# syshin1014/wssdl_bus

Hardware: AMD Instinct MI355X
Metric: images/sec (train step, 600x1000) (higher is better)
Workload: dtype f32; 1 GPU; resnet50_joint_b8; backbone=ResNet-50, image=600x1000, images_per_gpu=8, supervised_per_gpu=4, weak_per_gpu=4, mode=joint, parallelism=image-parallel dp1, RCCL grad all-reduce, sampling_rng=device, fused_rpn_softmax=True, padded_rois=False, miopen_find=True, miopen_find_db=wssdl_bus_amd/miopen_db (HIP.3_5_0_20250912-42-1199-g2584e35062), miopen_searched=True

## Files before the change

### wssdl_bus_amd/csrc/plumbing/rowbn.hip

```cpp
#include <hip/hip_runtime.h>
#include <stdint.h>
#include <type_traits>

#define PLUMB_API extern "C" __attribute__((visibility("default")))

namespace {

constexpr int BLOCK = 256;
constexpr int MAX_PARTIAL_BLOCKS = 1024;

typedef float float4v __attribute__((ext_vector_type(4)));

template <int MASK>
__device__ __forceinline__ unsigned mask_roi(long long r, int div) {
    return MASK == 2 ? (unsigned)r % (unsigned)div : (unsigned)r / (unsigned)div;
}

__device__ __forceinline__ float bn_affine(float x, float sc, float sh) { return __builtin_fmaf(x, sc, sh); }
__device__ __forceinline__ float bn_dx(float ka, float u, float k0, float k1, float x) {
    return __builtin_fmaf(-k1, x, __builtin_fmaf(ka, u, -k0));
}
__device__ __forceinline__ void dot_rows2(double &q, float v0, float w0, float v1, float w1) {
#pragma clang fp contract(off)
    const double p1 = (double)v1 * (double)w1;
    q += __builtin_fma((double)v0, (double)w0, p1);
}
__device__ __forceinline__ void dot_row(double &q, float v, float w) { q = __builtin_fma((double)v, (double)w, q); }
__device__ __forceinline__ void acc_rows2(double &s, double &q, float v0, float w0, float v1, float w1) {
    s += (double)v0 + (double)v1;
    dot_rows2(q, v0, w0, v1, w1);
}
__device__ __forceinline__ void acc_row(double &s, double &q, float v, float w) {
    s += (double)v;
    dot_row(q, v, w);
}

template <int MASK>
__device__ __forceinline__ bool row_live(const float *__restrict__ mask, long long r, int div) {
    return MASK ? mask[mask_roi<MASK>(r, div)] != 0.0f : true;
}

__device__ __forceinline__ float4v load4(const float *__restrict__ p, long long r, int C, int c4, bool on) {
    const float4v zero4 = {0, 0, 0, 0};
    return on ? reinterpret_cast<const float4v *>(p + (size_t)r * C)[c4] : zero4;
}

__device__ __forceinline__ void store4(float *__restrict__ p, long long r, int C, int c4, float4v v) {
    reinterpret_cast<float4v *>(p + (size_t)r * C)[c4] = v;
}

struct EntryGrad {
    const float *dys;
    const int *possel;
    int per, R;
};

template <bool ENTRY>
__device__ __forceinline__ float4v load_dy(const float *__restrict__ dy, const EntryGrad &e, long long r, int C, int c4,
                                           bool on = true) {
    const float4v zero4 = {0, 0, 0, 0};
    if (!on) return zero4;
    const float4v g = reinterpret_cast<const float4v *>(dy + (size_t)r * C)[c4];
    if (!ENTRY) return g;
    const unsigned roi = (unsigned)r / (unsigned)e.per, p = (unsigned)r - roi * (unsigned)e.per;
    const int slot = e.possel[p];
    float4v d = zero4;
    if (slot >= 0) d = reinterpret_cast<const float4v *>(e.dys + ((size_t)slot * e.R + roi) * C)[c4] + zero4;
    return g + d;
}

struct Slab {
    int C4, L, RS, lc, lr;
    long long r0, r1;
    __device__ __forceinline__ Slab(long long M, int C, long long rows_per_block) {
        C4 = C >> 2;
        L = C4 < BLOCK ? C4 : BLOCK;
        RS = BLOCK / L;
        lc = threadIdx.x % L;
        lr = threadIdx.x / L;
        r0 = (long long)blockIdx.x * rows_per_block;
        r1 = r0 + rows_per_block < M ? r0 + rows_per_block : M;
    }
};

__device__ __forceinline__ void slab_reduce(const Slab &b, int C, int c4, const double (&s)[4], const double (&q)[4],
                                            double (*red)[8], double *__restrict__ out) {
    const int t = threadIdx.x;
    __syncthreads();
#pragma unroll
    for (int j = 0; j < 4; ++j) { red[t][j] = s[j]; red[t][4 + j] = q[j]; }
    __syncthreads();
    if (b.lr == 0) {
#pragma unroll
        for (int j = 0; j < 4; ++j) {
            double ss = 0.0, qq = 0.0;
            for (int k = 0; k < b.RS; ++k) { ss += red[k * b.L + b.lc][j]; qq += red[k * b.L + b.lc][4 + j]; }
            out[c4 * 4 + j] = ss;
            out[C + c4 * 4 + j] = qq;
        }
    }
}

struct Term {
    float4v v, w, w2;
};

template <int MASK, class F>
__device__ __forceinline__ void slab_walk(const Slab &b, int C, const float *__restrict__ mask, int div, F &f,
                                          double (*red)[8], double *__restrict__ out,
                                          double *__restrict__ out2 = nullptr) {
    const int RS = b.RS;
    for (int cc = 0; cc * b.L < b.C4; ++cc) {
        const int c4 = cc * b.L + b.lc;
        double s[4] = {0, 0, 0, 0}, q[4] = {0, 0, 0, 0}, q2[4] = {0, 0, 0, 0};
        f.setup(c4);
        if (b.lr < RS) {
            long long r = b.r0 + b.lr;
#pragma unroll 1
            for (; r + RS < b.r1; r += 2 * RS) {
                const bool live0 = row_live<MASK>(mask, r, div), live1 = row_live<MASK>(mask, r + RS, div);
                if (!F::VISITS_DEAD && !live0 && !live1) continue;
                const typename F::Row a0 = f.load(r, c4, live0), a1 = f.load(r + RS, c4, live1);
                const Term t0 = f.finish(a0, r, c4, live0), t1 = f.finish(a1, r + RS, c4, live1);
#pragma unroll
                for (int j = 0; j < 4; ++j) {
                    const float v0 = live0 ? t0.v[j] : 0.0f, v1 = live1 ? t1.v[j] : 0.0f;
                    acc_rows2(s[j], q[j], v0, live0 ? t0.w[j] : 0.0f, v1, live1 ? t1.w[j] : 0.0f);
                    if (F::TWO_Q) dot_rows2(q2[j], v0, live0 ? t0.w2[j] : 0.0f, v1, live1 ? t1.w2[j] : 0.0f);
                }
            }
            for (; r < b.r1; r += RS) {
                const bool live = row_live<MASK>(mask, r, div);
                if (!F::VISITS_DEAD && !live) continue;
                const Term t = f.finish(f.load(r, c4, live), r, c4, live);
                if (live) {
#pragma unroll
                    for (int j = 0; j < 4; ++j) {
                        acc_row(s[j], q[j], t.v[j], t.w[j]);
                        if (F::TWO_Q) dot_row(q2[j], t.v[j], t.w2[j]);
                    }
                }
            }
        }
        slab_reduce(b, C, c4, s, q, red, out);
        if (F::TWO_Q) slab_reduce(b, C, c4, s, q2, red, out2);
    }
}

template <int MODE, bool RELU, bool ENTRY>
struct PartialCols {
    static constexpr bool VISITS_DEAD = false, TWO_Q = false;
    const float *x, *dy, *scale, *shift;
    int C;
    EntryGrad eg;
    float4v sc, sh;
    struct Row {
        float4v a, g;
    };
    __device__ __forceinline__ void setup(int c4) {
        if (MODE == 1 && RELU) {
            sc = reinterpret_cast<const float4v *>(scale)[c4];
            sh = reinterpret_cast<const float4v *>(shift)[c4];
        }
    }
    __device__ __forceinline__ Row load(long long r, int c4, bool live) const {
        Row w = {load4(x, r, C, c4, live), {0, 0, 0, 0}};
        if (MODE == 1) w.g = load_dy<ENTRY>(dy, eg, r, C, c4, live);
        return w;
    }
    __device__ __forceinline__ Term finish(const Row &w, long long, int, bool) const {
        Term t = {w.a, w.a, {0, 0, 0, 0}};
        if (MODE == 1) {
            t.v = w.g;
#pragma unroll
            for (int j = 0; j < 4; ++j)
                if (RELU && !(bn_affine(w.a[j], sc[j], sh[j]) > 0.0f)) t.v[j] = 0.0f;
        }
        return t;
    }
};

template <int MODE, bool RELU, int MASK, bool ENTRY = false>
__global__ __launch_bounds__(BLOCK) void rowbn_partial_kernel(
    const float *__restrict__ x, const float *__restrict__ dy, const float *__restrict__ scale,
    const float *__restrict__ shift, long long M, int C, long long rows_per_block,
    double *__restrict__ partial, const float *__restrict__ mask, int per, EntryGrad eg = EntryGrad()) {
    __shared__ double red[BLOCK][8];
    const Slab b(M, C, rows_per_block);
    PartialCols<MODE, RELU, ENTRY> f = {x, dy, scale, shift, C, eg};
    slab_walk<MASK>(b, C, mask, per, f, red, partial + (size_t)blockIdx.x * 2 * C);
}

constexpr int FIN_COLS = 16, FIN_GROUPS = 64;

__device__ __forceinline__ void finish_reduce(const double *__restrict__ partial, int nblocks, int C,
                                              int c, int grp, double (*red)[FIN_COLS][2], double &s,
                                              double &q) {
    double ss = 0.0, qq = 0.0;
    if (c < C)
        for (int b = grp; b < nblocks; b += FIN_GROUPS) {
            ss += partial[(size_t)b * 2 * C + c];
            qq += partial[(size_t)b * 2 * C + C + c];
        }
    red[grp][threadIdx.x % FIN_COLS][0] = ss;
    red[grp][threadIdx.x % FIN_COLS][1] = qq;
    __syncthreads();
    s = 0.0;
    q = 0.0;
    if (grp == 0)
        for (int g = 0; g < FIN_GROUPS; ++g) {
            s += red[g][threadIdx.x][0];
            q += red[g][threadIdx.x][1];
        }
}

__device__ __forceinline__ double live_rows(const float *__restrict__ mask, int n_rois, int per, long long M,
                                            double *scratch ) {
    if (!mask) return (double)M;
    double c = 0.0;
    for (int i = threadIdx.x; i < n_rois; i += FIN_COLS * FIN_GROUPS) c += mask[i] != 0.0f ? 1.0 : 0.0;
    __syncthreads();
    scratch[threadIdx.x] = c;
    __syncthreads();
    double t = 0.0;
    for (int i = 0; i < FIN_COLS * FIN_GROUPS; ++i) t += scratch[i];
    __syncthreads();
    t *= (double)per;
    return t < 1.0 ? 1.0 : t;
}

struct Running {
    float *mean, *var;
    float momentum;
    long long *batches;
};

__device__ __forceinline__ float running_update(float r, float stat, double unbias, double mom) {
#pragma clang fp contract(off)
    const double t = (double)stat * unbias;
    const double d = t - (double)r;
    const double p = mom * d;
    return (float)((double)r + p);
}

__global__ __launch_bounds__(FIN_COLS * FIN_GROUPS) void rowbn_fwd_finish_kernel(
    const double *__restrict__ partial, int nblocks, int C, long long M,
    const float *__restrict__ weight, const float *__restrict__ bias, float eps,
    float *__restrict__ mean, float *__restrict__ var, float *__restrict__ rstd,
    float *__restrict__ scale, float *__restrict__ shift, const float *__restrict__ mask, int n_rois, int per,
    float *__restrict__ count, Running run) {
    __shared__ double red[FIN_GROUPS][FIN_COLS][2];
    const int grp = threadIdx.x / FIN_COLS;
    const int c = blockIdx.x * FIN_COLS + threadIdx.x % FIN_COLS;
    const double Mn = live_rows(mask, n_rois, per, M, &red[0][0][0]);
    if (blockIdx.x == 0 && threadIdx.x == 0) {
        if (count) count[0] = (float)Mn;
        if (run.batches) run.batches[0] = run.batches[0] + 1;
    }
    double s, q;
    finish_reduce(partial, nblocks, C, c, grp, red, s, q);
    if (grp != 0 || c >= C) return;
    const double mu = s / Mn;
    double v = q / Mn - mu * mu;
    if (v < 0.0) v = 0.0;
    const float rs = (float)(1.0 / sqrt(v + (double)eps));
    const float scl = rs * weight[c];
    mean[c] = (float)mu;
    var[c] = (float)v;
    rstd[c] = rs;
    scale[c] = scl;
    shift[c] = bias[c] - (float)mu * scl;
    const double mom = (double)run.momentum;
    if (run.mean) run.mean[c] = running_update(run.mean[c], (float)mu, 1.0, mom);
    if (run.var) run.var[c] = running_update(run.var[c], (float)v, Mn / (Mn - 1.0 > 1.0 ? Mn - 1.0 : 1.0), mom);
}

__global__ __launch_bounds__(FIN_COLS * FIN_GROUPS) void rowbn_bwd_finish_kernel(
    const double *__restrict__ partial, int nblocks, int C, long long M,
    const float *__restrict__ weight, const float *__restrict__ mean,
    const float *__restrict__ rstd, float *__restrict__ dweight, float *__restrict__ dbias,
    float *__restrict__ coef, const float *__restrict__ mask, int n_rois, int per) {
    __shared__ double red[FIN_GROUPS][FIN_COLS][2];
    const int grp = threadIdx.x / FIN_COLS;
    const int c = blockIdx.x * FIN_COLS + threadIdx.x % FIN_COLS;
    const double Mn = live_rows(mask, n_rois, per, M, &red[0][0][0]);
    double sg, sgx;
    finish_reduce(partial, nblocks, C, c, grp, red, sg, sgx);
    if (grp != 0 || c >= C) return;
    const double mu = mean[c], rs = rstd[c], w = weight[c];
    const double sum_g_xhat = (sgx - mu * sg) * rs;
    const double a = w * rs;
    const double k1 = a * rs * sum_g_xhat / Mn;
    const double k0 = a * sg / Mn - k1 * mu;
    dweight[c] = (float)sum_g_xhat;
    dbias[c] = (float)sg;
    coef[c] = (float)a;
    coef[C + c] = (float)k0;
    coef[2 * C + c] = (float)k1;
}

template <bool RELU, int MASK>
__global__ __launch_bounds__(BLOCK) void rowbn_apply_fwd_kernel(
    const float *__restrict__ x, const float *__restrict__ scale, const float *__restrict__ shift,
    long long total4, int C4, float *__restrict__ y, const float *__restrict__ mask, int per) {
    for (long long i = (long long)blockIdx.x * BLOCK + threadIdx.x; i < total4;
         i += (long long)gridDim.x * BLOCK) {
        const int c4 = (int)(i % C4);
        if (MASK && mask[mask_roi<MASK>(i / C4, per)] == 0.0f) {
            const float4v zero4 = {0, 0, 0, 0};
            reinterpret_cast<float4v *>(y)[i] = zero4;
            continue;
        }
        const float4v a = reinterpret_cast<const float4v *>(x)[i];
        const float4v sc = reinterpret_cast<const float4v *>(scale)[c4];
        const float4v sh = reinterpret_cast<const float4v *>(shift)[c4];
        float4v o;
#pragma unroll
        for (int j = 0; j < 4; ++j) {
            float v = bn_affine(a[j], sc[j], sh[j]);
            if (RELU) v = v > 0.0f ? v : 0.0f;
            o[j] = v;
        }
        reinterpret_cast<float4v *>(y)[i] = o;
    }
}

template <bool RELU, int MASK, bool ENTRY = false>
__global__ __launch_bounds__(BLOCK) void rowbn_apply_bwd_kernel(
    const float *__restrict__ x, const float *__restrict__ dy, const float *__restrict__ scale,
    const float *__restrict__ shift, const float *__restrict__ coef, long long total4, int C4,
    float *__restrict__ dx, const float *__restrict__ mask, int per, EntryGrad eg = EntryGrad()) {
    const int C = C4 * 4;
    for (long long i = (long long)blockIdx.x * BLOCK + threadIdx.x; i < total4;
         i += (long long)gridDim.x * BLOCK) {
        const int c4 = (int)(i % C4);
        if (MASK && mask[mask_roi<MASK>(i / C4, per)] == 0.0f) {
            const float4v zero4 = {0, 0, 0, 0};
            reinterpret_cast<float4v *>(dx)[i] = zero4;
            continue;
        }
        const float4v a = reinterpret_cast<const float4v *>(x)[i];
        const float4v g = ENTRY ? load_dy<true>(dy, eg, i / C4, C, c4) : reinterpret_cast<const float4v *>(dy)[i];
        const float4v ka = reinterpret_cast<const float4v *>(coef)[c4];
        const float4v k0 = reinterpret_cast<const float4v *>(coef + C)[c4];
        const float4v k1 = reinterpret_cast<const float4v *>(coef + 2 * C)[c4];
        float4v sc = {0, 0, 0, 0}, sh = {0, 0, 0, 0};
        if (RELU) {
            sc = reinterpret_cast<const float4v *>(scale)[c4];
            sh = reinterpret_cast<const float4v *>(shift)[c4];
        }
        float4v o;
#pragma unroll
        for (int j = 0; j < 4; ++j) {
            float u = g[j];
            if (RELU && !(bn_affine(a[j], sc[j], sh[j]) > 0.0f)) u = 0.0f;
            o[j] = bn_dx(ka[j], u, k0[j], k1[j], a[j]);
        }
        reinterpret_cast<float4v *>(dx)[i] = o;
    }
}


__device__ __forceinline__ void acc_rows2_loose(double &s, double &q, float v0, float w0, float v1, float w1) {
    s += (double)v0 + (double)v1;
    q += (double)v0 * (double)w0 + (double)v1 * (double)w1;
}
__device__ __forceinline__ void acc_row_loose(double &s, double &q, float v, float w) {
    s += (double)v;
    q += (double)v * (double)w;
}

template <bool DUAL, int MASK>
__global__ __launch_bounds__(BLOCK) void rowbn_join_fwd_kernel(
    const float *__restrict__ x3, const float *__restrict__ sc3, const float *__restrict__ sh3,
    const float *__restrict__ other, const float *__restrict__ sco, const float *__restrict__ sho, long long M,
    int C, long long rows_per_block, float *__restrict__ out, double *__restrict__ partial,
    const float *__restrict__ mask, int div) {
    __shared__ double red[BLOCK][8];
    const Slab b(M, C, rows_per_block);
    double *pout = partial + (size_t)blockIdx.x * 2 * C;
    for (int cc = 0; cc * b.L < b.C4; ++cc) {
        const int c4 = cc * b.L + b.lc;
        double s[4] = {0, 0, 0, 0}, q[4] = {0, 0, 0, 0};
        const float4v k3 = reinterpret_cast<const float4v *>(sc3)[c4], h3 = reinterpret_cast<const float4v *>(sh3)[c4];
        float4v ko = {0, 0, 0, 0}, ho = {0, 0, 0, 0};
        if (DUAL) {
            ko = reinterpret_cast<const float4v *>(sco)[c4];
            ho = reinterpret_cast<const float4v *>(sho)[c4];
        }
        auto join = [&](float a, float o, int j, bool live) {
            const float t = live ? bn_affine(a, k3[j], h3[j]) : 0.0f;
            const float u = DUAL ? (live ? bn_affine(o, ko[j], ho[j]) : 0.0f) : o;
            return t + u;
        };
        if (b.lr < b.RS) {
            const int RS = b.RS;
            long long r = b.r0 + b.lr;
#pragma unroll 1
            for (; r + RS < b.r1; r += 2 * RS) {
                const bool live0 = row_live<MASK>(mask, r, div), live1 = row_live<MASK>(mask, r + RS, div);
                const float4v a0 = load4(x3, r, C, c4, live0), a1 = load4(x3, r + RS, C, c4, live1);
                const float4v o0 = load4(other, r, C, c4, !DUAL || live0), o1 = load4(other, r + RS, C, c4, !DUAL || live1);
                float4v y0, y1;
#pragma unroll
                for (int j = 0; j < 4; ++j) {
                    y0[j] = join(a0[j], o0[j], j, live0);
                    y1[j] = join(a1[j], o1[j], j, live1);
                    const float v0 = live0 ? y0[j] : 0.0f, v1 = live1 ? y1[j] : 0.0f;
                    acc_rows2_loose(s[j], q[j], v0, v0, v1, v1);
                }
                store4(out, r, C, c4, y0);
                store4(out, r + RS, C, c4, y1);
            }
            for (; r < b.r1; r += RS) {
                const bool live0 = row_live<MASK>(mask, r, div);
                const float4v a0 = load4(x3, r, C, c4, live0), o0 = load4(other, r, C, c4, !DUAL || live0);
                float4v y0;
#pragma unroll
                for (int j = 0; j < 4; ++j) {
                    y0[j] = join(a0[j], o0[j], j, live0);
                    if (live0) acc_row_loose(s[j], q[j], y0[j], y0[j]);
                }
                store4(out, r, C, c4, y0);
            }
        }
        slab_reduce(b, C, c4, s, q, red, pout);
    }
}

template <bool DUAL, bool RES>
struct JoinBwdCols {
    static constexpr bool VISITS_DEAD = true, TWO_Q = DUAL;
    const float *xo, *dy, *scn, *shn, *coef, *dres, *x3, *xs;
    float *g;
    int C;
    float4v sc, sh, ka, k0, k1;
    struct Row {
        float4v x, d, e, a, b;
    };
    __device__ __forceinline__ void setup(int c4) {
        sc = reinterpret_cast<const float4v *>(scn)[c4];
        sh = reinterpret_cast<const float4v *>(shn)[c4];
        ka = reinterpret_cast<const float4v *>(coef)[c4];
        k0 = reinterpret_cast<const float4v *>(coef + C)[c4];
        k1 = reinterpret_cast<const float4v *>(coef + 2 * C)[c4];
    }
    __device__ __forceinline__ Row load(long long r, int c4, bool live) const {
        return {load4(xo, r, C, c4, live), load4(dy, r, C, c4, live), load4(dres, r, C, c4, RES),
                load4(x3, r, C, c4, live), load4(xs, r, C, c4, DUAL && live)};
    }
    __device__ __forceinline__ Term finish(const Row &w, long long r, int c4, bool live) const {
        float4v o;
#pragma unroll
        for (int j = 0; j < 4; ++j) {
            float u = w.d[j];
            if (!(bn_affine(w.x[j], sc[j], sh[j]) > 0.0f)) u = 0.0f;
            const float dx = live ? bn_dx(ka[j], u, k0[j], k1[j], w.x[j]) : 0.0f;
            o[j] = RES ? dx + w.e[j] : dx;
        }
        store4(g, r, C, c4, o);
        return {o, w.a, w.b};
    }
};

template <bool DUAL, bool RES, int MASK>
__global__ __launch_bounds__(BLOCK) void rowbn_join_bwd_kernel(
    const float *__restrict__ xo, const float *__restrict__ dy, const float *__restrict__ scn,
    const float *__restrict__ shn, const float *__restrict__ coef, const float *__restrict__ dres,
    const float *__restrict__ x3, const float *__restrict__ xs, long long M, int C, long long rows_per_block,
    float *__restrict__ g, double *__restrict__ partial3, double *__restrict__ partials,
    const float *__restrict__ mask, int div) {
    __shared__ double red[BLOCK][8];
    const Slab b(M, C, rows_per_block);
    JoinBwdCols<DUAL, RES> f = {xo, dy, scn, shn, coef, dres, x3, xs, g, C};
    slab_walk<MASK>(b, C, mask, div, f, red, partial3 + (size_t)blockIdx.x * 2 * C,
                    DUAL ? partials + (size_t)blockIdx.x * 2 * C : nullptr);
}

template <int MASK>
__global__ __launch_bounds__(BLOCK) void rowbn_apply_bwd_dual_kernel(
    const float *__restrict__ x3, const float *__restrict__ xs, const float *__restrict__ g,
    const float *__restrict__ coef3, const float *__restrict__ coefs, long long total4, int C4,
    float *__restrict__ dx3, float *__restrict__ dxs, const float *__restrict__ mask, int div) {
    const int C = C4 * 4;
    for (long long i = (long long)blockIdx.x * BLOCK + threadIdx.x; i < total4;
         i += (long long)gridDim.x * BLOCK) {
        const int c4 = (int)(i % C4);
        if (MASK && mask[mask_roi<MASK>(i / C4, div)] == 0.0f) {
            const float4v zero4 = {0, 0, 0, 0};
            reinterpret_cast<float4v *>(dx3)[i] = zero4;
            reinterpret_cast<float4v *>(dxs)[i] = zero4;
            continue;
        }
        const float4v a = reinterpret_cast<const float4v *>(x3)[i];
        const float4v e = reinterpret_cast<const float4v *>(xs)[i];
        const float4v u = reinterpret_cast<const float4v *>(g)[i];
        const float4v ka3 = reinterpret_cast<const float4v *>(coef3)[c4], kas = reinterpret_cast<const float4v *>(coefs)[c4];
        const float4v k03 = reinterpret_cast<const float4v *>(coef3 + C)[c4], k0s = reinterpret_cast<const float4v *>(coefs + C)[c4];
        const float4v k13 = reinterpret_cast<const float4v *>(coef3 + 2 * C)[c4], k1s = reinterpret_cast<const float4v *>(coefs + 2 * C)[c4];
        float4v o3, os;
#pragma unroll
        for (int j = 0; j < 4; ++j) {
            o3[j] = bn_dx(ka3[j], u[j], k03[j], k13[j], a[j]);
            os[j] = bn_dx(kas[j], u[j], k0s[j], k1s[j], e[j]);
        }
        reinterpret_cast<float4v *>(dx3)[i] = o3;
        reinterpret_cast<float4v *>(dxs)[i] = os;
    }
}

inline int partial_blocks(long long M, int C) {
    const int C4 = C / 4;
    const int L = C4 < BLOCK ? C4 : BLOCK;
    const int RS = BLOCK / L;
    long long want = (M + (long long)RS * 16 - 1) / ((long long)RS * 16);
    if (want < 1) want = 1;
    return (int)(want < MAX_PARTIAL_BLOCKS ? want : MAX_PARTIAL_BLOCKS);
}

inline bool shape_ok(long long M, int C) {
    if (M < 1 || C < 4 || (C & 3)) return false;
    const int C4 = C / 4;
    return C4 <= BLOCK ? (BLOCK % C4 == 0) : (C4 % BLOCK == 0);
}

inline int apply_grid(long long total4) {
    long long b = (total4 + BLOCK - 1) / BLOCK;
    return (int)(b < 65536 ? b : 65536);
}

}

PLUMB_API size_t wsplumb_rowbn_workspace_bytes(long long M, int C) {
    if (!shape_ok(M, C)) return 0;
    return (size_t)partial_blocks(M, C) * 2 * (size_t)C * sizeof(double);
}

PLUMB_API int wsplumb_rowbn_supported(long long M, int C) { return shape_ok(M, C) ? 1 : 0; }

PLUMB_API size_t wsplumb_rowbn_join_workspace_bytes(long long M, int C) {
    return 2 * wsplumb_rowbn_workspace_bytes(M, C);
}

namespace {

struct Geom {
    hipStream_t st;
    long long M, rpb, total4;
    int C, nb;
    const float *mask;
    int mode, div;
    int n_rois, per;
    double *p0, *p1;
};

inline int make_geom(Geom &g, long long M, int C, const float *mask, int n_rois, int per, bool pos_major, bool grouped,
                     bool args_ok, void *workspace, size_t workspace_bytes, int n_partials, void *stream) {
    if (!args_ok || M < 1 || C < 4 || (C & 3)) return 1;
    if (n_partials && (!shape_ok(M, C) || workspace_bytes < n_partials * wsplumb_rowbn_workspace_bytes(M, C))) return 1;
    if (pos_major && !mask) return 1;
    if ((mask || grouped) && (per < 1 || n_rois < 1 || (long long)n_rois * per != M || M > 0x7fffffffLL)) return 1;
    g.st = static_cast<hipStream_t>(stream);
    g.M = M;
    g.C = C;
    g.nb = n_partials ? partial_blocks(M, C) : 0;
    g.rpb = n_partials ? (M + g.nb - 1) / g.nb : 0;
    g.total4 = M * (C / 4);
    g.mask = mask;
    g.mode = mask ? (pos_major ? 2 : 1) : 0;
    g.div = mask ? (pos_major ? n_rois : per) : 1;
    g.n_rois = n_rois;
    g.per = per;
    g.p0 = static_cast<double *>(workspace);
    g.p1 = g.p0 + (size_t)g.nb * 2 * C;
    return 0;
}

template <auto... Vs, class T, class F>
inline void pick(T v, F &&f) {
    (void)((v == Vs && (f(std::integral_constant<decltype(Vs), Vs>{}), true)) || ...);
}

inline void launch_sums(const Geom &g, const float *x, double *partial) {
    pick<0, 1, 2>(g.mode, [&](auto MASK) {
        hipLaunchKernelGGL((rowbn_partial_kernel<0, false, MASK>), dim3(g.nb), dim3(BLOCK), 0, g.st, x, nullptr, nullptr,
                           nullptr, g.M, g.C, g.rpb, partial, g.mask, g.div);
    });
}

inline void launch_grad_sums(const Geom &g, const float *x, const float *dy, const float *scale, const float *shift,
                             bool relu, const EntryGrad *eg, double *partial) {
    if (eg)
        pick<0, 1>(g.mode, [&](auto MASK) {
            hipLaunchKernelGGL((rowbn_partial_kernel<1, true, MASK, true>), dim3(g.nb), dim3(BLOCK), 0, g.st, x, dy, scale,
                               shift, g.M, g.C, g.rpb, partial, g.mask, g.div, *eg);
        });
    else
        pick<false, true>(relu, [&](auto RELU) {
            pick<0, 1, 2>(g.mode, [&](auto MASK) {
                hipLaunchKernelGGL((rowbn_partial_kernel<1, RELU, MASK>), dim3(g.nb), dim3(BLOCK), 0, g.st, x, dy, scale,
                                   shift, g.M, g.C, g.rpb, partial, g.mask, g.div);
            });
        });
}

inline void launch_fwd_finish(const Geom &g, const double *partial, const float *weight, const float *bias, float eps,
                              float *mean, float *var, float *rstd, float *scale, float *shift, float *count,
                              Running run) {
    hipLaunchKernelGGL(rowbn_fwd_finish_kernel, dim3((g.C + FIN_COLS - 1) / FIN_COLS), dim3(FIN_COLS * FIN_GROUPS), 0,
                       g.st, partial, g.nb, g.C, g.M, weight, bias, eps, mean, var, rstd, scale, shift, g.mask, g.n_rois,
                       g.per, g.mask ? count : nullptr, run);
}

inline void launch_fwd_finish(const Geom &g, const double *partial, const float *weight, const float *bias, float eps,
                              float *stats, float *count, Running run) {
    const int C = g.C;
    launch_fwd_finish(g, partial, weight, bias, eps, stats, stats + C, stats + 2 * C, stats + 3 * C, stats + 4 * C, count,
                      run);
}

inline void launch_bwd_finish(const Geom &g, const double *partial, const float *weight, const float *mean,
                              const float *rstd, float *dweight, float *dbias, float *coef) {
    hipLaunchKernelGGL(rowbn_bwd_finish_kernel, dim3((g.C + FIN_COLS - 1) / FIN_COLS), dim3(FIN_COLS * FIN_GROUPS), 0,
                       g.st, partial, g.nb, g.C, g.M, weight, mean, rstd, dweight, dbias, coef, g.mask, g.n_rois, g.per);
}

inline void launch_apply_fwd(const Geom &g, const float *x, const float *scale, const float *shift, bool relu, float *y) {
    pick<false, true>(relu, [&](auto RELU) {
        pick<0, 1, 2>(g.mode, [&](auto MASK) {
            hipLaunchKernelGGL((rowbn_apply_fwd_kernel<RELU, MASK>), dim3(apply_grid(g.total4)), dim3(BLOCK), 0, g.st, x,
                               scale, shift, g.total4, g.C / 4, y, g.mask, g.div);
        });
    });
}

inline void launch_apply_bwd(const Geom &g, const float *x, const float *dy, const float *scale, const float *shift,
                             const float *coef, bool relu, const EntryGrad *eg, float *dx) {
    if (eg)
        pick<0, 1>(g.mode, [&](auto MASK) {
            hipLaunchKernelGGL((rowbn_apply_bwd_kernel<true, MASK, true>), dim3(apply_grid(g.total4)), dim3(BLOCK), 0, g.st,
                               x, dy, scale, shift, coef, g.total4, g.C / 4, dx, g.mask, g.div, *eg);
        });
    else
        pick<false, true>(relu, [&](auto RELU) {
            pick<0, 1, 2>(g.mode, [&](auto MASK) {
                hipLaunchKernelGGL((rowbn_apply_bwd_kernel<RELU, MASK>), dim3(apply_grid(g.total4)), dim3(BLOCK), 0, g.st,
                                   x, dy, scale, shift, coef, g.total4, g.C / 4, dx, g.mask, g.div);
            });
        });
}

inline int launched() { return hipGetLastError() == hipSuccess ? 0 : 3; }

int backward_impl(const Geom &g, const float *x, const float *dy, const EntryGrad *eg, const float *weight,
                  const float *mean, const float *rstd, const float *scale, const float *shift, bool relu, float *dx,
                  float *dweight, float *dbias, float *coef) {
    launch_grad_sums(g, x, dy, scale, shift, relu, eg, g.p0);
    launch_bwd_finish(g, g.p0, weight, mean, rstd, dweight, dbias, coef);
    launch_apply_bwd(g, x, dy, scale, shift, coef, relu, eg, dx);
    return launched();
}

}

PLUMB_API int wsplumb_rowbn_forward(const float *x, long long M, int C, const float *weight, const float *bias,
                                    float eps, int relu, const float *mask, int n_rois, int per, int pos_major,
                                    float *y, float *mean, float *var, float *rstd, float *scale, float *shift,
                                    float *count, void *workspace, size_t workspace_bytes, void *stream,
                                    float *running_mean, float *running_var, float momentum,
                                    long long *num_batches_tracked) {
    Geom g;
    if (make_geom(g, M, C, mask, n_rois, per, pos_major != 0, false, !mask || count, workspace, workspace_bytes, 1,
                  stream))
        return 1;
    launch_sums(g, x, g.p0);
    launch_fwd_finish(g, g.p0, weight, bias, eps, mean, var, rstd, scale, shift, count,
                      Running{running_mean, running_var, momentum, num_batches_tracked});
    launch_apply_fwd(g, x, scale, shift, relu != 0, y);
    return launched();
}

PLUMB_API int wsplumb_rowbn_apply(const float *x, long long M, int C, const float *scale,
                                  const float *shift, int relu, float *y, void *stream) {
    Geom g;
    if (make_geom(g, M, C, nullptr, 0, 1, false, false, true, nullptr, 0, 0, stream)) return 1;
    launch_apply_fwd(g, x, scale, shift, relu != 0, y);
    return launched();
}

PLUMB_API int wsplumb_rowbn_backward(const float *x, const float *dy, long long M, int C, const float *weight,
                                     const float *mean, const float *rstd, const float *scale, const float *shift,
                                     int relu, const float *mask, int n_rois, int per, int pos_major, float *dx,
                                     float *dweight, float *dbias, float *coef, void *workspace,
                                     size_t workspace_bytes, void *stream) {
    Geom g;
    if (make_geom(g, M, C, mask, n_rois, per, pos_major != 0, false, true, workspace, workspace_bytes, 1, stream))
        return 1;
    return backward_impl(g, x, dy, nullptr, weight, mean, rstd, scale, shift, relu != 0, dx, dweight, dbias, coef);
}

PLUMB_API int wsplumb_rowbn_backward_entry(const float *x, const float *dy, const float *dys, const int *possel,
                                           int n_slots, long long M, int C, const float *weight, const float *mean,
                                           const float *rstd, const float *scale, const float *shift,
                                           const float *mask, int n_rois, int per, float *dx, float *dweight,
                                           float *dbias, float *coef, void *workspace, size_t workspace_bytes,
                                           void *stream) {
    Geom g;
    if (make_geom(g, M, C, mask, n_rois, per, false, true, dys && possel && n_slots >= 1 && n_slots <= per, workspace,
                  workspace_bytes, 1, stream))
        return 1;
    const EntryGrad eg = {dys, possel, per, n_rois};
    return backward_impl(g, x, dy, &eg, weight, mean, rstd, scale, shift, true, dx, dweight, dbias, coef);
}


PLUMB_API int wsplumb_rowbn_join_forward(const float *x3, const float *other, long long M, int C,
                                         const float *weight3, const float *bias3, float eps3,
                                         const float *weight_s, const float *bias_s, float eps_s,
                                         const float *weight_n, const float *bias_n, float eps_n,
                                         const float *mask, int n_rois, int per, float *out, float *y,
                                         float *stats3, float *stats_s, float *stats_n, float *count,
                                         void *workspace, size_t workspace_bytes, void *stream,
                                         float *const *running, const float *momentum,
                                         long long *const *batches) {
    const bool dual = weight_s != nullptr;
    Geom g;
    if (make_geom(g, M, C, mask, n_rois, per, mask != nullptr, false, (!mask || count) && (!dual || (bias_s && stats_s)),
                  workspace, workspace_bytes, 2, stream))
        return 1;
    Running run[3] = {};
    for (int k = 0; k < 3; ++k) {
        if (running) { run[k].mean = running[2 * k]; run[k].var = running[2 * k + 1]; }
        if (momentum) run[k].momentum = momentum[k];
        if (batches) run[k].batches = batches[k];
    }
    launch_sums(g, x3, g.p0);
    launch_fwd_finish(g, g.p0, weight3, bias3, eps3, stats3, nullptr, run[0]);
    if (dual) {
        launch_sums(g, other, g.p0);
        launch_fwd_finish(g, g.p0, weight_s, bias_s, eps_s, stats_s, nullptr, run[1]);
    }
    const float *sco = dual ? stats_s + 3 * C : nullptr, *sho = dual ? stats_s + 4 * C : nullptr;
    pick<false, true>(dual, [&](auto DUAL) {
        pick<0, 2>(g.mode, [&](auto MASK) {
            hipLaunchKernelGGL((rowbn_join_fwd_kernel<DUAL, MASK>), dim3(g.nb), dim3(BLOCK), 0, g.st, x3, stats3 + 3 * C,
                               stats3 + 4 * C, other, sco, sho, M, C, g.rpb, out, g.p0, mask, g.div);
        });
    });
    launch_fwd_finish(g, g.p0, weight_n, bias_n, eps_n, stats_n, count, run[2]);
    launch_apply_fwd(g, out, stats_n + 3 * C, stats_n + 4 * C, true, y);
    return launched();
}

PLUMB_API int wsplumb_rowbn_join_backward(const float *out, const float *dy, const float *dres, const float *x3,
                                          const float *xs, long long M, int C, const float *weight_n,
                                          const float *stats_n, const float *weight3, const float *stats3,
                                          const float *weight_s, const float *stats_s, const float *mask,
                                          int n_rois, int per, float *gout, float *dx3, float *dxs, float *dwb_n,
                                          float *dwb3, float *dwb_s, float *coef, void *workspace,
                                          size_t workspace_bytes, void *stream) {
    const bool dual = xs != nullptr;
    Geom g;
    if (make_geom(g, M, C, mask, n_rois, per, mask != nullptr, false, !dual || (weight_s && stats_s && dxs && dwb_s),
                  workspace, workspace_bytes, 2, stream))
        return 1;
    float *coef_n = coef, *coef3 = coef + 3 * C, *coefs = coef + 6 * C;
    const float *scn = stats_n + 3 * C, *shn = stats_n + 4 * C;
    launch_grad_sums(g, out, dy, scn, shn, true, nullptr, g.p0);
    launch_bwd_finish(g, g.p0, weight_n, stats_n, stats_n + 2 * C, dwb_n, dwb_n + C, coef_n);
    pick<false, true>(dual, [&](auto DUAL) {
        pick<false, true>(dres != nullptr, [&](auto RES) {
            pick<0, 2>(g.mode, [&](auto MASK) {
                hipLaunchKernelGGL((rowbn_join_bwd_kernel<DUAL, RES, MASK>), dim3(g.nb), dim3(BLOCK), 0, g.st, out, dy, scn,
                                   shn, coef_n, dres, x3, xs, M, C, g.rpb, gout, g.p0, g.p1, mask, g.div);
            });
        });
    });
    launch_bwd_finish(g, g.p0, weight3, stats3, stats3 + 2 * C, dwb3, dwb3 + C, coef3);
    if (dual) {
        launch_bwd_finish(g, g.p1, weight_s, stats_s, stats_s + 2 * C, dwb_s, dwb_s + C, coefs);
        pick<0, 2>(g.mode, [&](auto MASK) {
            hipLaunchKernelGGL((rowbn_apply_bwd_dual_kernel<MASK>), dim3(apply_grid(g.total4)), dim3(BLOCK), 0, g.st, x3, xs,
                               gout, coef3, coefs, g.total4, C / 4, dx3, dxs, mask, g.div);
        });
    } else {
        launch_apply_bwd(g, x3, gout, nullptr, nullptr, coef3, false, nullptr, dx3);
    }
    return launched();
}
```

Measured before the change: 55.51 images/s.

## Restructure row-BN slab walk into grid-strided tiles with batched loads and 2D grid

Row-BN partial-sum kernels switch from contiguous per-block row ranges with a serial column loop to a 2D grid (column chunks on blockIdx.y) and grid-strided tiles of several rows per thread. Loads for a tile are issued together using clamped safe row addresses instead of predicated loads, and the mask for the next tile is prefetched. Entry-gradient gathers are split into index and load phases. The join forward kernel is folded into the shared walker, the finish reduction batches partial loads, and the live-row count uses a wave shuffle reduction. The aim is more memory-level parallelism and less latency exposure, at the cost of extra register pressure and reads of dead rows.

```diff
diff --git a/wssdl_bus_amd/csrc/plumbing/rowbn.hip b/wssdl_bus_amd/csrc/plumbing/rowbn.hip
--- a/wssdl_bus_amd/csrc/plumbing/rowbn.hip
+++ b/wssdl_bus_amd/csrc/plumbing/rowbn.hip
@@ -8,6 +8,7 @@
 
 constexpr int BLOCK = 256;
 constexpr int MAX_PARTIAL_BLOCKS = 1024;
+constexpr int PARTIAL_ROWS = 4, JOIN_FWD_ROWS = 4, JOIN_BWD_ROWS = 2;
 
 typedef float float4v __attribute__((ext_vector_type(4)));
 
@@ -40,9 +41,12 @@
     return MASK ? mask[mask_roi<MASK>(r, div)] != 0.0f : true;
 }
 
-__device__ __forceinline__ float4v load4(const float *__restrict__ p, long long r, int C, int c4, bool on) {
+template <bool EN = true>
+__device__ __forceinline__ float4v load4(const float *__restrict__ p, long long r, long long rsafe, int C, int c4,
+                                         bool on) {
     const float4v zero4 = {0, 0, 0, 0};
-    return on ? reinterpret_cast<const float4v *>(p + (size_t)r * C)[c4] : zero4;
+    if (!EN) return zero4;
+    return reinterpret_cast<const float4v *>(p + (size_t)(on ? r : rsafe) * C)[c4];
 }
 
 __device__ __forceinline__ void store4(float *__restrict__ p, long long r, int C, int c4, float4v v) {
@@ -69,17 +73,35 @@
     return g + d;
 }
 
+__device__ __forceinline__ int entry_slot(const EntryGrad &e, long long r, long long rsafe, bool on) {
+    return e.possel[(unsigned)(on ? r : rsafe) % (unsigned)e.per];
+}
+__device__ __forceinline__ float4v entry_dys(const float *__restrict__ dy, const EntryGrad &e, int slot, long long r,
+                                             long long rsafe, int C, int c4, bool on) {
+    const float4v zero4 = {0, 0, 0, 0};
+    const unsigned roi = (unsigned)(on ? r : rsafe) / (unsigned)e.per;
+    const bool has = slot >= 0;
+    const float *drow = has ? e.dys + ((size_t)slot * e.R + roi) * C : dy + (size_t)rsafe * C;
+    const float4v d = reinterpret_cast<const float4v *>(drow)[c4];
+    return has ? d + zero4 : zero4;
+}
+
+constexpr int TILE_ROWS = 4;
+
 struct Slab {
-    int C4, L, RS, lc, lr;
-    long long r0, r1;
-    __device__ __forceinline__ Slab(long long M, int C, long long rows_per_block) {
+    int C4, L, RS, lc, lr, c4;
+    long long r0, r1, tile, stride;
+    __device__ __forceinline__ Slab(long long M, int C) {
         C4 = C >> 2;
         L = C4 < BLOCK ? C4 : BLOCK;
         RS = BLOCK / L;
         lc = threadIdx.x % L;
         lr = threadIdx.x / L;
-        r0 = (long long)blockIdx.x * rows_per_block;
-        r1 = r0 + rows_per_block < M ? r0 + rows_per_block : M;
+        c4 = blockIdx.y * L + lc;
+        tile = (long long)TILE_ROWS * RS;
+        stride = (long long)gridDim.x * tile;
+        r0 = (long long)blockIdx.x * tile;
+        r1 = M;
     }
 };
 
@@ -105,57 +127,122 @@
     float4v v, w, w2;
 };
 
+template <int MASK, int N>
+__device__ __forceinline__ void rows_mask(const Slab &b, const float *__restrict__ mask, int div, long long r,
+                                          float (&m)[N]) {
+#pragma unroll
+    for (int k = 0; k < N; ++k) {
+        const long long rk = r + k * b.RS;
+        m[k] = MASK ? mask[mask_roi<MASK>(rk < b.r1 ? rk : b.r1 - 1, div)] : 1.0f;
+    }
+}
+
+template <int MASK, int N, bool AHEAD, class F>
+__device__ __forceinline__ void walk_rows(const Slab &b, int C, const float *__restrict__ mask, int div, F &f,
+                                          long long r, long long rnext, const bool (&live)[N], float (&next)[N],
+                                          double (&s)[4],
+                                          double (&q)[4], double (&q2)[4]) {
+    const int RS = b.RS, c4 = b.c4;
+    bool any = false;
+#pragma unroll
+    for (int k = 0; k < N; ++k) any |= live[k];
+    if (!F::VISITS_DEAD && !any) {
+        if (AHEAD) rows_mask<MASK, N>(b, mask, div, rnext, next);
+        return;
+    }
+    typename F::Row a[N];
+#pragma unroll
+    for (int k = 0; k < N; ++k) f.index(a[k], r + k * RS, b.r0, live[k]);
+#pragma unroll
+    for (int k = 0; k < N; ++k) f.load(a[k], r + k * RS, b.r0, c4, live[k]);
+#pragma unroll
+    for (int k = 0; k < N; ++k) f.load_indexed(a[k], r + k * RS, b.r0, c4, live[k]);
+    if (AHEAD) rows_mask<MASK, N>(b, mask, div, rnext, next);
+    __builtin_amdgcn_sched_barrier(0);
+    if (N == 1) {
+        const Term t = f.finish(a[0], r, c4, live[0]);
+        if (live[0]) {
+#pragma unroll
+            for (int j = 0; j < 4; ++j) {
+                acc_row(s[j], q[j], t.v[j], t.w[j]);
+                if (F::TWO_Q) dot_row(q2[j], t.v[j], t.w2[j]);
+            }
+        }
+        return;
+    }
+#pragma unroll
+    for (int k = 0; k + 1 < N; k += 2) {
+        const bool live0 = live[k], live1 = live[k + 1];
+        const Term t0 = f.finish(a[k], r + k * RS, c4, live0), t1 = f.finish(a[k + 1], r + (k + 1) * RS, c4, live1);
+#pragma unroll
+        for (int j = 0; j < 4; ++j) {
+            const float v0 = live0 ? t0.v[j] : 0.0f, v1 = live1 ? t1.v[j] : 0.0f;
+            acc_rows2(s[j], q[j], v0, live0 ? t0.w[j] : 0.0f, v1, live1 ? t1.w[j] : 0.0f);
+            if (F::TWO_Q) dot_rows2(q2[j], v0, live0 ? t0.w2[j] : 0.0f, v1, live1 ? t1.w2[j] : 0.0f);
+        }
+    }
+}
+
 template <int MASK, class F>
 __device__ __forceinline__ void slab_walk(const Slab &b, int C, const float *__restrict__ mask, int div, F &f,
                                           double (*red)[8], double *__restrict__ out,
                                           double *__restrict__ out2 = nullptr) {
+    constexpr int N = F::ROWS;
+    static_assert(N >= 2 && N % 2 == 0 && TILE_ROWS % N == 0, "rows per step: pairs, a whole number of steps per tile");
     const int RS = b.RS;
-    for (int cc = 0; cc * b.L < b.C4; ++cc) {
-        const int c4 = cc * b.L + b.lc;
-        double s[4] = {0, 0, 0, 0}, q[4] = {0, 0, 0, 0}, q2[4] = {0, 0, 0, 0};
-        f.setup(c4);
-        if (b.lr < RS) {
-            long long r = b.r0 + b.lr;
+    double s[4] = {0, 0, 0, 0}, q[4] = {0, 0, 0, 0}, q2[4] = {0, 0, 0, 0};
+    f.setup(b.c4);
+    long long base = b.r0, r = b.r0 + b.lr;
+    if (base < b.r1) {
+        bool live[N];
+        float next[N], none1[1], none2[2];
+        rows_mask<MASK, N>(b, mask, div, r, next);
+#pragma unroll
+        for (int k = 0; k < N; ++k) live[k] = next[k] != 0.0f;
 #pragma unroll 1
-            for (; r + RS < b.r1; r += 2 * RS) {
-                const bool live0 = row_live<MASK>(mask, r, div), live1 = row_live<MASK>(mask, r + RS, div);
-                if (!F::VISITS_DEAD && !live0 && !live1) continue;
-                const typename F::Row a0 = f.load(r, c4, live0), a1 = f.load(r + RS, c4, live1);
-                const Term t0 = f.finish(a0, r, c4, live0), t1 = f.finish(a1, r + RS, c4, live1);
-#pragma unroll
-                for (int j = 0; j < 4; ++j) {
-                    const float v0 = live0 ? t0.v[j] : 0.0f, v1 = live1 ? t1.v[j] : 0.0f;
-                    acc_rows2(s[j], q[j], v0, live0 ? t0.w[j] : 0.0f, v1, live1 ? t1.w[j] : 0.0f);
-                    if (F::TWO_Q) dot_rows2(q2[j], v0, live0 ? t0.w2[j] : 0.0f, v1, live1 ? t1.w2[j] : 0.0f);
+        for (; base + b.tile <= b.r1; base += b.stride, r += b.stride) {
+#pragma unroll
+            for (int h = 0; h < TILE_ROWS / N; ++h) {
+                const long long rh = r + (long long)h * N * RS;
+                walk_rows<MASK, N, true>(b, C, mask, div, f, rh, h + 1 < TILE_ROWS / N ? rh + N * RS : r + b.stride, live,
+                                         next, s, q, q2);
+#pragma unroll
+                for (int k = 0; k < N; ++k) live[k] = next[k] != 0.0f;
+            }
+        }
+        if (base < b.r1) {
+            long long cnt = r < b.r1 ? (b.r1 - r + RS - 1) / RS : 0;
+#pragma unroll
+            for (int p = 0; p < TILE_ROWS / 2; ++p)
+                if (cnt >= 2) {
+                    rows_mask<MASK, 2>(b, mask, div, r, none2);
+                    const bool l2[2] = {none2[0] != 0.0f, none2[1] != 0.0f};
+                    walk_rows<MASK, 2, false>(b, C, mask, div, f, r, r, l2, none2, s, q, q2);
+                    r += 2 * RS;
+                    cnt -= 2;
                 }
+            if (cnt >= 1) {
+                rows_mask<MASK, 1>(b, mask, div, r, none1);
+                const bool l1[1] = {none1[0] != 0.0f};
+                walk_rows<MASK, 1, false>(b, C, mask, div, f, r, r, l1, none1, s, q, q2);
             }
-            for (; r < b.r1; r += RS) {
-                const bool live = row_live<MASK>(mask, r, div);
-                if (!F::VISITS_DEAD && !live) continue;
-                const Term t = f.finish(f.load(r, c4, live), r, c4, live);
-                if (live) {
-#pragma unroll
-                    for (int j = 0; j < 4; ++j) {
-                        acc_row(s[j], q[j], t.v[j], t.w[j]);
-                        if (F::TWO_Q) dot_row(q2[j], t.v[j], t.w2[j]);
-                    }
-                }
-            }
-        }
-        slab_reduce(b, C, c4, s, q, red, out);
-        if (F::TWO_Q) slab_reduce(b, C, c4, s, q2, red, out2);
-    }
+        }
+    }
+    slab_reduce(b, C, b.c4, s, q, red, out);
+    if (F::TWO_Q) slab_reduce(b, C, b.c4, s, q2, red, out2);
 }
 
 template <int MODE, bool RELU, bool ENTRY>
 struct PartialCols {
     static constexpr bool VISITS_DEAD = false, TWO_Q = false;
+    static constexpr int ROWS = PARTIAL_ROWS;
     const float *x, *dy, *scale, *shift;
     int C;
     EntryGrad eg;
     float4v sc, sh;
     struct Row {
-        float4v a, g;
+        float4v a, g, d;
+        int slot;
     };
     __device__ __forceinline__ void setup(int c4) {
         if (MODE == 1 && RELU) {
@@ -163,15 +250,20 @@
             sh = reinterpret_cast<const float4v *>(shift)[c4];
         }
     }
-    __device__ __forceinline__ Row load(long long r, int c4, bool live) const {
-        Row w = {load4(x, r, C, c4, live), {0, 0, 0, 0}};
-        if (MODE == 1) w.g = load_dy<ENTRY>(dy, eg, r, C, c4, live);
-        return w;
+    __device__ __forceinline__ void index(Row &w, long long r, long long rsafe, bool live) const {
+        if (ENTRY) w.slot = entry_slot(eg, r, rsafe, live);
+    }
+    __device__ __forceinline__ void load(Row &w, long long r, long long rsafe, int c4, bool live) const {
+        w.a = load4(x, r, rsafe, C, c4, live);
+        if (MODE == 1) w.g = load4(dy, r, rsafe, C, c4, live);
+    }
+    __device__ __forceinline__ void load_indexed(Row &w, long long r, long long rsafe, int c4, bool live) const {
+        if (ENTRY) w.d = entry_dys(dy, eg, w.slot, r, rsafe, C, c4, live);
     }
     __device__ __forceinline__ Term finish(const Row &w, long long, int, bool) const {
         Term t = {w.a, w.a, {0, 0, 0, 0}};
         if (MODE == 1) {
-            t.v = w.g;
+            t.v = ENTRY ? w.g + w.d : w.g;
 #pragma unroll
             for (int j = 0; j < 4; ++j)
                 if (RELU && !(bn_affine(w.a[j], sc[j], sh[j]) > 0.0f)) t.v[j] = 0.0f;
@@ -183,24 +275,36 @@
 template <int MODE, bool RELU, int MASK, bool ENTRY = false>
 __global__ __launch_bounds__(BLOCK) void rowbn_partial_kernel(
     const float *__restrict__ x, const float *__restrict__ dy, const float *__restrict__ scale,
-    const float *__restrict__ shift, long long M, int C, long long rows_per_block,
+    const float *__restrict__ shift, long long M, int C,
     double *__restrict__ partial, const float *__restrict__ mask, int per, EntryGrad eg = EntryGrad()) {
     __shared__ double red[BLOCK][8];
-    const Slab b(M, C, rows_per_block);
+    const Slab b(M, C);
     PartialCols<MODE, RELU, ENTRY> f = {x, dy, scale, shift, C, eg};
     slab_walk<MASK>(b, C, mask, per, f, red, partial + (size_t)blockIdx.x * 2 * C);
 }
 
-constexpr int FIN_COLS = 16, FIN_GROUPS = 64;
+constexpr int FIN_COLS = 16, FIN_GROUPS = 64, FIN_BATCH = 16;
 
 __device__ __forceinline__ void finish_reduce(const double *__restrict__ partial, int nblocks, int C,
                                               int c, int grp, double (*red)[FIN_COLS][2], double &s,
                                               double &q) {
     double ss = 0.0, qq = 0.0;
     if (c < C)
-        for (int b = grp; b < nblocks; b += FIN_GROUPS) {
-            ss += partial[(size_t)b * 2 * C + c];
-            qq += partial[(size_t)b * 2 * C + C + c];
+        for (int b0 = grp; b0 < nblocks; b0 += FIN_GROUPS * FIN_BATCH) {
+            double ps[FIN_BATCH], pq[FIN_BATCH];
+#pragma unroll
+            for (int k = 0; k < FIN_BATCH; ++k) {
+                const int b = b0 + k * FIN_GROUPS;
+                const double *row = partial + (size_t)(b < nblocks ? b : b0) * 2 * C;
+                ps[k] = row[c];
+                pq[k] = row[C + c];
+            }
+#pragma unroll
+            for (int k = 0; k < FIN_BATCH; ++k)
+                if (b0 + k * FIN_GROUPS < nblocks) {
+                    ss += ps[k];
+                    qq += pq[k];
+                }
         }
     red[grp][threadIdx.x % FIN_COLS][0] = ss;
     red[grp][threadIdx.x % FIN_COLS][1] = qq;
@@ -217,14 +321,20 @@
 __device__ __forceinline__ double live_rows(const float *__restrict__ mask, int n_rois, int per, long long M,
                                             double *scratch ) {
     if (!mask) return (double)M;
-    double c = 0.0;
-    for (int i = threadIdx.x; i < n_rois; i += FIN_COLS * FIN_GROUPS) c += mask[i] != 0.0f ? 1.0 : 0.0;
+    constexpr int WAVES = FIN_COLS * FIN_GROUPS / 64;
+    int *wave_sum = reinterpret_cast<int *>(scratch);
+    int c = 0;
+    for (int i = threadIdx.x; i < n_rois; i += FIN_COLS * FIN_GROUPS) c += mask[i] != 0.0f ? 1 : 0;
+#pragma unroll
+    for (int off = 32; off > 0; off >>= 1) c += __shfl_xor(c, off, 64);
     __syncthreads();
-    scratch[threadIdx.x] = c;
+    if ((threadIdx.x & 63) == 0) wave_sum[threadIdx.x >> 6] = c;
     __syncthreads();
-    double t = 0.0;
-    for (int i = 0; i < FIN_COLS * FIN_GROUPS; ++i) t += scratch[i];
+    int n = 0;
+#pragma unroll
+    for (int i = 0; i < WAVES; ++i) n += wave_sum[i];
     __syncthreads();
+    double t = (double)n;
     t *= (double)per;
     return t < 1.0 ? 1.0 : t;
 }
@@ -361,76 +471,60 @@
 }
 
 
-__device__ __forceinline__ void acc_rows2_loose(double &s, double &q, float v0, float w0, float v1, float w1) {
-    s += (double)v0 + (double)v1;
-    q += (double)v0 * (double)w0 + (double)v1 * (double)w1;
-}
-__device__ __forceinline__ void acc_row_loose(double &s, double &q, float v, float w) {
-    s += (double)v;
-    q += (double)v * (double)w;
-}
+template <bool DUAL>
+struct JoinFwdCols {
+    static constexpr bool VISITS_DEAD = true, TWO_Q = false;
+    static constexpr int ROWS = JOIN_FWD_ROWS;
+    const float *x3, *sc3, *sh3, *other, *sco, *sho;
+    float *out;
+    int C;
+    float4v k3, h3, ko, ho;
+    struct Row {
+        float4v a, o;
+    };
+    __device__ __forceinline__ void setup(int c4) {
+        k3 = reinterpret_cast<const float4v *>(sc3)[c4];
+        h3 = reinterpret_cast<const float4v *>(sh3)[c4];
+        if (DUAL) {
+            ko = reinterpret_cast<const float4v *>(sco)[c4];
+            ho = reinterpret_cast<const float4v *>(sho)[c4];
+        }
+    }
+    __device__ __forceinline__ void index(Row &, long long, long long, bool) const {}
+    __device__ __forceinline__ void load(Row &w, long long r, long long rsafe, int c4, bool live) const {
+        w.a = load4(x3, r, rsafe, C, c4, live);
+        w.o = load4(other, r, rsafe, C, c4, !DUAL || live);
+    }
+    __device__ __forceinline__ void load_indexed(Row &, long long, long long, int, bool) const {}
+    __device__ __forceinline__ Term finish(const Row &w, long long r, int c4, bool live) const {
+        float4v y;
+#pragma unroll
+        for (int j = 0; j < 4; ++j) {
+            const float t = live ? bn_affine(w.a[j], k3[j], h3[j]) : 0.0f;
+            const float u = DUAL ? (live ? bn_affine(w.o[j], ko[j], ho[j]) : 0.0f) : w.o[j];
+            y[j] = t + u;
+        }
+        store4(out, r, C, c4, y);
+        return {y, y, {0, 0, 0, 0}};
+    }
+};
 
 template <bool DUAL, int MASK>
 __global__ __launch_bounds__(BLOCK) void rowbn_join_fwd_kernel(
     const float *__restrict__ x3, const float *__restrict__ sc3, const float *__restrict__ sh3,
     const float *__restrict__ other, const float *__restrict__ sco, const float *__restrict__ sho, long long M,
-    int C, long long rows_per_block, float *__restrict__ out, double *__restrict__ partial,
+    int C, float *__restrict__ out, double *__restrict__ partial,
     const float *__restrict__ mask, int div) {
     __shared__ double red[BLOCK][8];
-    const Slab b(M, C, rows_per_block);
-    double *pout = partial + (size_t)blockIdx.x * 2 * C;
-    for (int cc = 0; cc * b.L < b.C4; ++cc) {
-        const int c4 = cc * b.L + b.lc;
-        double s[4] = {0, 0, 0, 0}, q[4] = {0, 0, 0, 0};
-        const float4v k3 = reinterpret_cast<const float4v *>(sc3)[c4], h3 = reinterpret_cast<const float4v *>(sh3)[c4];
-        float4v ko = {0, 0, 0, 0}, ho = {0, 0, 0, 0};
-        if (DUAL) {
-            ko = reinterpret_cast<const float4v *>(sco)[c4];
-            ho = reinterpret_cast<const float4v *>(sho)[c4];
-        }
-        auto join = [&](float a, float o, int j, bool live) {
-            const float t = live ? bn_affine(a, k3[j], h3[j]) : 0.0f;
-            const float u = DUAL ? (live ? bn_affine(o, ko[j], ho[j]) : 0.0f) : o;
-            return t + u;
-        };
-        if (b.lr < b.RS) {
-            const int RS = b.RS;
-            long long r = b.r0 + b.lr;
-#pragma unroll 1
-            for (; r + RS < b.r1; r += 2 * RS) {
-                const bool live0 = row_live<MASK>(mask, r, div), live1 = row_live<MASK>(mask, r + RS, div);
-                const float4v a0 = load4(x3, r, C, c4, live0), a1 = load4(x3, r + RS, C, c4, live1);
-                const float4v o0 = load4(other, r, C, c4, !DUAL || live0), o1 = load4(other, r + RS, C, c4, !DUAL || live1);
-                float4v y0, y1;
-#pragma unroll
-                for (int j = 0; j < 4; ++j) {
-                    y0[j] = join(a0[j], o0[j], j, live0);
-                    y1[j] = join(a1[j], o1[j], j, live1);
-                    const float v0 = live0 ? y0[j] : 0.0f, v1 = live1 ? y1[j] : 0.0f;
-                    acc_rows2_loose(s[j], q[j], v0, v0, v1, v1);
-                }
-                store4(out, r, C, c4, y0);
-                store4(out, r + RS, C, c4, y1);
-            }
-            for (; r < b.r1; r += RS) {
-                const bool live0 = row_live<MASK>(mask, r, div);
-                const float4v a0 = load4(x3, r, C, c4, live0), o0 = load4(other, r, C, c4, !DUAL || live0);
-                float4v y0;
-#pragma unroll
-                for (int j = 0; j < 4; ++j) {
-                    y0[j] = join(a0[j], o0[j], j, live0);
-                    if (live0) acc_row_loose(s[j], q[j], y0[j], y0[j]);
-                }
-                store4(out, r, C, c4, y0);
-            }
-        }
-        slab_reduce(b, C, c4, s, q, red, pout);
-    }
+    const Slab b(M, C);
+    JoinFwdCols<DUAL> f = {x3, sc3, sh3, other, sco, sho, out, C};
+    slab_walk<MASK>(b, C, mask, div, f, red, partial + (size_t)blockIdx.x * 2 * C);
 }
 
 template <bool DUAL, bool RES>
 struct JoinBwdCols {
     static constexpr bool VISITS_DEAD = true, TWO_Q = DUAL;
+    static constexpr int ROWS = JOIN_BWD_ROWS;
     const float *xo, *dy, *scn, *shn, *coef, *dres, *x3, *xs;
     float *g;
     int C;
@@ -445,10 +539,15 @@
         k0 = reinterpret_cast<const float4v *>(coef + C)[c4];
         k1 = reinterpret_cast<const float4v *>(coef + 2 * C)[c4];
     }
-    __device__ __forceinline__ Row load(long long r, int c4, bool live) const {
-        return {load4(xo, r, C, c4, live), load4(dy, r, C, c4, live), load4(dres, r, C, c4, RES),
-                load4(x3, r, C, c4, live), load4(xs, r, C, c4, DUAL && live)};
-    }
+    __device__ __forceinline__ void index(Row &, long long, long long, bool) const {}
+    __device__ __forceinline__ void load(Row &w, long long r, long long rsafe, int c4, bool live) const {
+        w.x = load4(xo, r, rsafe, C, c4, live);
+        w.d = load4(dy, r, rsafe, C, c4, live);
+        w.e = load4<RES>(dres, r, rsafe, C, c4, true);
+        w.a = load4(x3, r, rsafe, C, c4, live);
+        w.b = load4<DUAL>(xs, r, rsafe, C, c4, live);
+    }
+    __device__ __forceinline__ void load_indexed(Row &, long long, long long, int, bool) const {}
     __device__ __forceinline__ Term finish(const Row &w, long long r, int c4, bool live) const {
         float4v o;
 #pragma unroll
@@ -467,11 +566,11 @@
 __global__ __launch_bounds__(BLOCK) void rowbn_join_bwd_kernel(
     const float *__restrict__ xo, const float *__restrict__ dy, const float *__restrict__ scn,
     const float *__restrict__ shn, const float *__restrict__ coef, const float *__restrict__ dres,
-    const float *__restrict__ x3, const float *__restrict__ xs, long long M, int C, long long rows_per_block,
+    const float *__restrict__ x3, const float *__restrict__ xs, long long M, int C,
     float *__restrict__ g, double *__restrict__ partial3, double *__restrict__ partials,
     const float *__restrict__ mask, int div) {
     __shared__ double red[BLOCK][8];
-    const Slab b(M, C, rows_per_block);
+    const Slab b(M, C);
     JoinBwdCols<DUAL, RES> f = {xo, dy, scn, shn, coef, dres, x3, xs, g, C};
     slab_walk<MASK>(b, C, mask, div, f, red, partial3 + (size_t)blockIdx.x * 2 * C,
                     DUAL ? partials + (size_t)blockIdx.x * 2 * C : nullptr);
@@ -524,6 +623,11 @@
     return C4 <= BLOCK ? (BLOCK % C4 == 0) : (C4 % BLOCK == 0);
 }
 
+inline dim3 slab_grid(int nb, int C) {
+    const int C4 = C / 4;
+    return dim3(nb, C4 > BLOCK ? C4 / BLOCK : 1);
+}
+
 inline int apply_grid(long long total4) {
     long long b = (total4 + BLOCK - 1) / BLOCK;
     return (int)(b < 65536 ? b : 65536);
@@ -546,7 +650,7 @@
 
 struct Geom {
     hipStream_t st;
-    long long M, rpb, total4;
+    long long M, total4;
     int C, nb;
     const float *mask;
     int mode, div;
@@ -564,7 +668,6 @@
     g.M = M;
     g.C = C;
     g.nb = n_partials ? partial_blocks(M, C) : 0;
-    g.rpb = n_partials ? (M + g.nb - 1) / g.nb : 0;
     g.total4 = M * (C / 4);
     g.mask = mask;
     g.mode = mask ? (pos_major ? 2 : 1) : 0;
@@ -583,8 +686,8 @@
 
 inline void launch_sums(const Geom &g, const float *x, double *partial) {
     pick<0, 1, 2>(g.mode, [&](auto MASK) {
-        hipLaunchKernelGGL((rowbn_partial_kernel<0, false, MASK>), dim3(g.nb), dim3(BLOCK), 0, g.st, x, nullptr, nullptr,
-                           nullptr, g.M, g.C, g.rpb, partial, g.mask, g.div);
+        hipLaunchKernelGGL((rowbn_partial_kernel<0, false, MASK>), slab_grid(g.nb, g.C), dim3(BLOCK), 0, g.st, x, nullptr, nullptr,
+                           nullptr, g.M, g.C, partial, g.mask, g.div);
     });
 }
 
@@ -592,14 +695,14 @@
                              bool relu, const EntryGrad *eg, double *partial) {
     if (eg)
         pick<0, 1>(g.mode, [&](auto MASK) {
-            hipLaunchKernelGGL((rowbn_partial_kernel<1, true, MASK, true>), dim3(g.nb), dim3(BLOCK), 0, g.st, x, dy, scale,
-                               shift, g.M, g.C, g.rpb, partial, g.mask, g.div, *eg);
+            hipLaunchKernelGGL((rowbn_partial_kernel<1, true, MASK, true>), slab_grid(g.nb, g.C), dim3(BLOCK), 0, g.st, x, dy, scale,
+                               shift, g.M, g.C, partial, g.mask, g.div, *eg);
         });
     else
         pick<false, true>(relu, [&](auto RELU) {
             pick<0, 1, 2>(g.mode, [&](auto MASK) {
-                hipLaunchKernelGGL((rowbn_partial_kernel<1, RELU, MASK>), dim3(g.nb), dim3(BLOCK), 0, g.st, x, dy, scale,
-                                   shift, g.M, g.C, g.rpb, partial, g.mask, g.div);
+                hipLaunchKernelGGL((rowbn_partial_kernel<1, RELU, MASK>), slab_grid(g.nb, g.C), dim3(BLOCK), 0, g.st, x, dy, scale,
+                                   shift, g.M, g.C, partial, g.mask, g.div);
             });
         });
 }
@@ -743,8 +846,8 @@
     const float *sco = dual ? stats_s + 3 * C : nullptr, *sho = dual ? stats_s + 4 * C : nullptr;
     pick<false, true>(dual, [&](auto DUAL) {
         pick<0, 2>(g.mode, [&](auto MASK) {
-            hipLaunchKernelGGL((rowbn_join_fwd_kernel<DUAL, MASK>), dim3(g.nb), dim3(BLOCK), 0, g.st, x3, stats3 + 3 * C,
-                               stats3 + 4 * C, other, sco, sho, M, C, g.rpb, out, g.p0, mask, g.div);
+            hipLaunchKernelGGL((rowbn_join_fwd_kernel<DUAL, MASK>), slab_grid(g.nb, g.C), dim3(BLOCK), 0, g.st, x3, stats3 + 3 * C,
+                               stats3 + 4 * C, other, sco, sho, M, C, out, g.p0, mask, g.div);
         });
     });
     launch_fwd_finish(g, g.p0, weight_n, bias_n, eps_n, stats_n, count, run[2]);
@@ -771,8 +874,8 @@
     pick<false, true>(dual, [&](auto DUAL) {
         pick<false, true>(dres != nullptr, [&](auto RES) {
             pick<0, 2>(g.mode, [&](auto MASK) {
-                hipLaunchKernelGGL((rowbn_join_bwd_kernel<DUAL, RES, MASK>), dim3(g.nb), dim3(BLOCK), 0, g.st, out, dy, scn,
-                                   shn, coef_n, dres, x3, xs, M, C, g.rpb, gout, g.p0, g.p1, mask, g.div);
+                hipLaunchKernelGGL((rowbn_join_bwd_kernel<DUAL, RES, MASK>), slab_grid(g.nb, g.C), dim3(BLOCK), 0, g.st, out, dy, scn,
+                                   shn, coef_n, dres, x3, xs, M, C, gout, g.p0, g.p1, mask, g.div);
             });
         });
     });
```

Result: no change. 55.95 images/s, median of 6 (+0.8%).
